# xswang/xflow

Hardware: NVIDIA H100
Metric: training examples/sec (higher is better)
Workload: dtype f32

## Files before the change

xflow_b200/csrc/kernels.cu:

```cuda
#include <cuda_runtime.h>
#include <stdint.h>
#include <stdlib.h>

#include "kernels.h"
#include "table.cuh"

__global__ void xf_k_fill(uint8_t* base, uint64_t cap, uint32_t stride, int lazy) {
  const uint64_t chunks_per_row = stride / 16;
  const uint64_t total = cap * chunks_per_row;
  for (uint64_t c = (uint64_t)blockIdx.x * blockDim.x + threadIdx.x; c < total;
       c += (uint64_t)gridDim.x * blockDim.x) {
    uint64_t r = c / chunks_per_row;
    uint32_t q = (uint32_t)(c % chunks_per_row);
    uint4 v = make_uint4(0, 0, 0, 0);
    if (q == 0) {
      v.x = 0xFFFFFFFFu; v.y = 0xFFFFFFFFu;
      if (!lazy) v.w = XF_NEG_ZERO_BITS;
    }
    *reinterpret_cast<uint4*>(base + r * stride + (uint64_t)q * 16) = v;
  }
}

template <int VEC>
__device__ __forceinline__ void xf_ldv(const float* p, float (&o)[VEC]) {
  if (VEC == 4) { float4 t = __ldcg(reinterpret_cast<const float4*>(p)); o[0] = t.x; o[1 % VEC] = t.y; o[2 % VEC] = t.z; o[3 % VEC] = t.w; }
  else if (VEC == 2) { float2 t = __ldcg(reinterpret_cast<const float2*>(p)); o[0] = t.x; o[1 % VEC] = t.y; }
  else { o[0] = __ldcg(p); }
}
template <int VEC>
__device__ __forceinline__ void xf_stv(float* p, const float (&o)[VEC]) {
  if (VEC == 4) *reinterpret_cast<float4*>(p) = make_float4(o[0], o[1 % VEC], o[2 % VEC], o[3 % VEC]);
  else if (VEC == 2) *reinterpret_cast<float2*>(p) = make_float2(o[0], o[1 % VEC]);
  else *p = o[0];
}
template <int VEC, bool SLOTG, bool STAMP>
__global__ void __launch_bounds__(256)
xf_k_update(XfTableView t, const uint32_t* __restrict__ slots, uint64_t n, int tps, double rows,
            const float* __restrict__ gw, const float* __restrict__ gv, int part,
            unsigned long long* __restrict__ live_total, const uint32_t* __restrict__ n_dev,
            const uint32_t* __restrict__ rows_dev, uint32_t extra_base, uint32_t extra_n,
            const float* __restrict__ v0_side, XfStampView sv) {
  __shared__ unsigned int s_live;
  if (threadIdx.x == 0) s_live = 0;
  __syncthreads();
  uint64_t n_head = n;
  if (n_dev != nullptr) {
    n_head = min((uint64_t)__ldg(n_dev), (uint64_t)extra_base);
    n = n_head + extra_n;
    rows = (double)__ldg(rows_dev);
  }
  unsigned int live_acc = 0;
  const int K = t.K;
  const unsigned lane = threadIdx.x & 31u;
  const uint64_t gwarp = ((uint64_t)blockIdx.x * blockDim.x + threadIdx.x) >> 5;
  const uint64_t nwarps = ((uint64_t)gridDim.x * blockDim.x) >> 5;
  const int q = (int)(lane & (unsigned)(tps - 1));
  const int gi = (int)(lane / (unsigned)tps);
  const int ngroups = 32 / tps;
  const int leader = (int)(lane & ~(unsigned)(tps - 1));
  const unsigned group_mask = (tps == 32) ? 0xffffffffu : (((1u << tps) - 1u) << leader);
  const int nchunk = K / VEC;

  for (uint64_t base = gwarp * 32; base < n; base += nwarps * 32) {
    const uint64_t e_fwd = base + lane;
    const uint64_t e_i = (SLOTG && e_fwd < n) ? (n - 1 - e_fwd) : e_fwd;
    const uint64_t e_phys = (e_i < n_head) ? e_i : (uint64_t)extra_base + (e_i - n_head);
    const uint32_t s_lane = (e_fwd < n) ? __ldcs(slots + e_phys) : 0xFFFFFFFFu;
    unsigned pend = __ballot_sync(0xffffffffu, s_lane != 0xFFFFFFFFu);
    if (live_total != nullptr && lane == 0) live_acc += __popc(pend);

    while (pend) {
      const int cnt = __popc(pend);
      const unsigned src = (gi < cnt) ? __fns(pend, 0, gi + 1) : 0u;
      const uint32_t s = __shfl_sync(0xffffffffu, s_lane, (int)src);
      const uint64_t i = __shfl_sync(0xffffffffu, (unsigned long long)e_i, (int)src);
      const uint64_t i_phys = __shfl_sync(0xffffffffu, (unsigned long long)e_phys, (int)src);
      uint8_t* rowp = (gi < cnt) ? xf_row(t, s) : nullptr;
      pend = (cnt <= ngroups) ? 0u : (pend & ~((2u << __fns(pend, 0, ngroups)) - 1u));

      const bool lat = K > 0 && (part & 2) && rowp != nullptr;
      float* vp = lat ? xf_row_v(rowp) : nullptr;
      float* nvp = lat ? xf_row_nv(rowp, K) : nullptr;
      float* zvp = lat ? xf_row_zv(rowp, K) : nullptr;
      float v0[VEC], n0[VEC], z0[VEC];
#pragma unroll
      for (int e = 0; e < VEC; ++e) { v0[e] = 0.f; n0[e] = 0.f; z0[e] = 0.f; }
      const bool has0 = lat && q < nchunk;
      if (has0) {
        xf_ldv<VEC>(vp + q * VEC, v0);
        if (t.opt == XF_OPT_FTRL) { xf_ldv<VEC>(nvp + q * VEC, n0); xf_ldv<VEC>(zvp + q * VEC, z0); }
      }
      float p0[VEC];
#pragma unroll
      for (int e = 0; e < VEC; ++e) p0[e] = 0.f;
      if (SLOTG && v0_side != nullptr && has0) {
        const uint64_t tok = (i_phys < (uint64_t)extra_base) ? i_phys : (uint64_t)__ldg(slots + i_phys + extra_n);
        xf_ldv<VEC>(v0_side + tok * (uint64_t)K + q * VEC, p0);
      }
      float ca0[VEC];
#pragma unroll
      for (int e = 0; e < VEC; ++e) ca0[e] = 0.f;
      if (SLOTG && t.canon && has0) xf_ldv<VEC>(xf_row_ca(t, rowp) + q * VEC, ca0);
      double accL = 0.0, accA = 0.0;
      if (SLOTG && has0) {
        const double2 a = __ldcg(reinterpret_cast<const double2*>(xf_row_acc(rowp, K)));
        accL = a.x;
        accA = a.y;
      }
      XfHead h;
      h.key = 0; h.flags = 0; h.w = h.n = h.z = 0.f; h.g = 0.0;
      if (q == 0 && rowp != nullptr) h = xf_load_head(rowp);
      const uint64_t key = __shfl_sync(group_mask, (unsigned long long)h.key, leader);
      const uint32_t flags = __shfl_sync(group_mask, h.flags, leader);
      if (rowp == nullptr) continue;

      if (q == 0) {
        if (!SLOTG) xf_apply_pending(t, h);
        if (part & 1) {
          const float g = SLOTG ? xf_div_rows((float)h.g, rows) : gw[i];
          xf_opt_coord(t, g, h.w, h.n, h.z);
        }
        if (SLOTG) h.g = -0.0;
        if (K > 0 && (part & 2)) h.flags |= XF_FLAG_V_READY;
        xf_store_head_t(t, rowp, h);
        if (STAMP) sv.stamp[s] = sv.now;
      }
      if (lat) {
        const bool ready = (flags & XF_FLAG_V_READY) != 0;
        for (int c = q; c < nchunk; c += tps) {
          const int k = c * VEC;
          float v[VEC], g[VEC], nn[VEC], zz[VEC];
#pragma unroll
          for (int e = 0; e < VEC; ++e) { v[e] = v0[e]; nn[e] = n0[e]; zz[e] = z0[e]; }
          if (c != q && ready) {
            xf_ldv<VEC>(vp + k, v);
            if (t.opt == XF_OPT_FTRL) { xf_ldv<VEC>(nvp + k, nn); xf_ldv<VEC>(zvp + k, zz); }
          }
          if (!ready) {
#pragma unroll
            for (int e = 0; e < VEC; ++e) { v[e] = xf_v_init(t, key, (uint32_t)(k + e)); nn[e] = 0.f; zz[e] = 0.f; }
          }
          if (SLOTG) {
            float vp0[VEC];
#pragma unroll
            for (int e = 0; e < VEC; ++e) vp0[e] = v[e];
            if (v0_side != nullptr) {
              if (c == q) {
#pragma unroll
                for (int e = 0; e < VEC; ++e) vp0[e] = p0[e];
              } else {
                const uint64_t tok = (i_phys < (uint64_t)extra_base) ? i_phys : (uint64_t)__ldg(slots + i_phys + extra_n);
                xf_ldv<VEC>(v0_side + tok * (uint64_t)K + k, vp0);
              }
            }
            if (t.canon) {
              float ca[VEC];
#pragma unroll
              for (int e = 0; e < VEC; ++e) ca[e] = ca0[e];
              if (c != q) xf_ldv<VEC>(xf_row_ca(t, rowp) + k, ca);
#pragma unroll
              for (int e = 0; e < VEC; ++e) g[e] = xf_div_rows((float)((double)ca[e] - (double)vp0[e] * accL), rows);
              const float zero[VEC] = {};
              xf_stv<VEC>(xf_row_ca(t, rowp) + k, zero);
            } else {
#pragma unroll
              for (int e = 0; e < VEC; ++e) g[e] = xf_div_rows((float)(accA - (double)vp0[e] * accL), rows);
            }
          } else {
#pragma unroll
            for (int e = 0; e < VEC; ++e) g[e] = gv[i * (uint64_t)K + k + e];
          }
          if (t.opt == XF_OPT_FTRL) {
#pragma unroll
            for (int e = 0; e < VEC; ++e) xf_ftrl_coord(t, g[e], v[e], nn[e], zz[e]);
            xf_stv<VEC>(nvp + k, nn);
            xf_stv<VEC>(zvp + k, zz);
          } else {
#pragma unroll
            for (int e = 0; e < VEC; ++e) xf_sgd_coord(t, g[e], v[e]);
          }
          xf_stv<VEC>(vp + k, v);
        }
        if (SLOTG) {
          __syncwarp(group_mask);
          if (q == 0) *reinterpret_cast<double2*>(xf_row_acc(rowp, K)) = make_double2(0.0, 0.0);
        }
      }
    }
  }
  if (live_total != nullptr) {
    if (lane == 0 && live_acc) atomicAdd(&s_live, live_acc);
    __syncthreads();
    if (threadIdx.x == 0 && s_live) atomicAdd_system(live_total, (unsigned long long)s_live);
  }
}

template <bool INSERT>
__global__ void xf_k_probe(XfTableView t, const uint64_t* __restrict__ keys, uint64_t n,
                           uint32_t* __restrict__ slots, float* __restrict__ w_out, XfStampView sv) {
  for (uint64_t i = (uint64_t)blockIdx.x * blockDim.x + threadIdx.x; i < n;
       i += (uint64_t)gridDim.x * blockDim.x) {
    XfHead h;
    h.w = 0.f;
    int64_t s = xf_probe<INSERT, true>(t, keys[i], &h, &sv);
    slots[i] = s >= 0 ? (uint32_t)s : 0xFFFFFFFFu;
    if (w_out) {
      if (s >= 0) xf_apply_pending(t, h);
      w_out[i] = s >= 0 ? h.w : 0.f;
    }
  }
}

__global__ void xf_k_gather_v(XfTableView t, const uint32_t* __restrict__ slots, const uint64_t* __restrict__ keys,
                              uint64_t n, float* __restrict__ v_out) {
  const int K = t.K;
  const uint64_t total = n * (uint64_t)K;
  for (uint64_t x = (uint64_t)blockIdx.x * blockDim.x + threadIdx.x; x < total;
       x += (uint64_t)gridDim.x * blockDim.x) {
    const uint64_t i = x / K;
    const int k = (int)(x % K);
    const uint32_t s = slots[i];
    float v = 0.f;
    if (s != 0xFFFFFFFFu) {
      const uint8_t* rowp = xf_row(t, s);
      const uint32_t flags = __ldcg(reinterpret_cast<const uint32_t*>(rowp + XF_OFF_FLAGS));
      v = (flags & XF_FLAG_V_READY) ? __ldcg(reinterpret_cast<const float*>(rowp + 32) + k)
                                    : xf_v_init(t, keys[i], (uint32_t)k);
    }
    v_out[x] = v;
  }
}

__global__ void xf_k_import(XfTableView t, const uint32_t* __restrict__ slots, uint64_t n,
                            const float* w, const float* nw, const float* zw, const float* v,
                            const float* nv, const float* zv) {
  const int K = t.K;
  const uint64_t per = (uint64_t)K + 1;
  const uint64_t total = n * per;
  for (uint64_t x = (uint64_t)blockIdx.x * blockDim.x + threadIdx.x; x < total;
       x += (uint64_t)gridDim.x * blockDim.x) {
    const uint64_t i = x / per;
    const int c = (int)(x % per);
    const uint32_t s = slots[i];
    if (s == 0xFFFFFFFFu) continue;
    uint8_t* rowp = xf_row(t, s);
    if (c == 0) {
      if (w) {
        if (t.lazy) {
          XfHead h;
          h.key = *reinterpret_cast<const uint64_t*>(rowp);
          h.w = w[i]; h.n = nw ? nw[i] : 0.f; h.z = zw ? zw[i] : 0.f; h.flags = 0u; h.g = 0.0;
          xf_lazy_store(t, rowp, h, true);
        } else {
          *reinterpret_cast<float2*>(rowp + XF_OFF_STATE) = make_float2(w[i], nw ? nw[i] : 0.f);
          *reinterpret_cast<float*>(rowp + XF_OFF_STATE + 8) = zw ? zw[i] : 0.f;
          *reinterpret_cast<unsigned long long*>(rowp + 8) = XF_NEG_ZERO_BITS64;
        }
      }
      if (v && K > 0) *reinterpret_cast<uint32_t*>(rowp + XF_OFF_FLAGS) = XF_FLAG_V_READY;
    } else if (v) {
      const int k = c - 1;
      xf_row_v(rowp)[k] = v[i * K + k];
      if (k == 0) *reinterpret_cast<double2*>(xf_row_acc(rowp, K)) = make_double2(0.0, 0.0);
      if (t.opt == XF_OPT_FTRL) {
        xf_row_nv(rowp, K)[k] = nv ? nv[i * K + k] : 0.f;
        xf_row_zv(rowp, K)[k] = zv ? zv[i * K + k] : 0.f;
      }
    }
  }
}

__global__ void xf_k_export(XfTableView t, const uint32_t* __restrict__ slots, const uint64_t* __restrict__ keys,
                            uint64_t n, float* w, float* nw, float* zw, float* v, float* nv, float* zv,
                            uint8_t* present) {
  const int K = t.K;
  const uint64_t per = (uint64_t)K + 1;
  const uint64_t total = n * per;
  for (uint64_t x = (uint64_t)blockIdx.x * blockDim.x + threadIdx.x; x < total;
       x += (uint64_t)gridDim.x * blockDim.x) {
    const uint64_t i = x / per;
    const int c = (int)(x % per);
    const uint32_t s = slots[i];
    const bool have = s != 0xFFFFFFFFu;
    const uint8_t* rowp = have ? xf_row(t, s) : nullptr;
    if (c == 0) {
      XfHead h;
      h.w = h.n = h.z = 0.f;
      if (have) {
        h = xf_load_head(rowp);
        xf_apply_pending(t, h);
      }
      if (present) present[i] = have ? 1 : 0;
      if (w) w[i] = h.w;
      if (nw) nw[i] = h.n;
      if (zw) zw[i] = h.z;
    } else if (v) {
      const int k = c - 1;
      float vv = 0.f, nn = 0.f, zz = 0.f;
      if (have) {
        const uint32_t flags = __ldcg(reinterpret_cast<const uint32_t*>(rowp + XF_OFF_FLAGS));
        if (flags & XF_FLAG_V_READY) {
          vv = __ldcg(reinterpret_cast<const float*>(rowp + 32) + k);
          if (t.opt == XF_OPT_FTRL) {
            nn = __ldcg(xf_row_nv(const_cast<uint8_t*>(rowp), K) + k);
            zz = __ldcg(xf_row_zv(const_cast<uint8_t*>(rowp), K) + k);
          }
        } else {
          vv = xf_v_init(t, keys[i], (uint32_t)k);
        }
      }
      v[i * K + k] = vv;
      if (nv) nv[i * K + k] = nn;
      if (zv) zv[i * K + k] = zz;
    }
  }
}

__global__ void xf_k_rehash(XfTableView src, XfTableView dst, XfKeep keep, const uint32_t* __restrict__ src_stamp,
                            uint32_t* __restrict__ dst_stamp) {
  const uint64_t cap = src.mask + 1;
  const uint32_t chunks = src.stride / 16;
  for (uint64_t r = (uint64_t)blockIdx.x * blockDim.x + threadIdx.x; r < cap;
       r += (uint64_t)gridDim.x * blockDim.x) {
    const uint8_t* srow = xf_row(src, r);
    uint4 a = *reinterpret_cast<const uint4*>(srow);
    uint64_t key = (uint64_t)a.x | ((uint64_t)a.y << 32);
    if (key == XF_EMPTY_KEY) continue;
    const uint32_t stamp = src_stamp != nullptr ? src_stamp[r] : 0u;
    if (src_stamp != nullptr && !xf_keeps(keep, stamp, key)) continue;
    XfHead h;
    int64_t s = xf_probe<true>(dst, key, &h);
    if (s < 0) continue;
    uint8_t* drow = xf_row(dst, (uint64_t)s);
    *reinterpret_cast<uint2*>(drow + 8) = make_uint2(a.z, a.w);
    for (uint32_t c = 1; c < chunks; ++c)
      *reinterpret_cast<uint4*>(drow + 16 * c) = *reinterpret_cast<const uint4*>(srow + 16 * c);
    if (dst_stamp != nullptr) dst_stamp[s] = stamp;
  }
}

__global__ void xf_k_list_keys(XfTableView t, uint64_t* keys_out, unsigned long long* count, uint64_t max_out) {
  const uint64_t cap = t.mask + 1;
  for (uint64_t r = (uint64_t)blockIdx.x * blockDim.x + threadIdx.x; r < cap;
       r += (uint64_t)gridDim.x * blockDim.x) {
    const uint64_t key = *reinterpret_cast<const uint64_t*>(xf_row(t, r));
    if (key == XF_EMPTY_KEY) continue;
    unsigned long long idx = atomicAdd(count, 1ull);
    if (idx < max_out) keys_out[idx] = key;
  }
}

static int g_sm_count = 0;
int xf_sms() {
  if (g_sm_count == 0) {
    int dev = 0;
    cudaGetDevice(&dev);
    cudaDeviceGetAttribute(&g_sm_count, cudaDevAttrMultiProcessorCount, dev);
    if (g_sm_count <= 0) g_sm_count = 132;
  }
  return g_sm_count;
}
int xf_grid_for(uint64_t work_items, int block, int blocks_per_sm) {
  uint64_t want = (work_items + block - 1) / block;
  uint64_t cap = (uint64_t)xf_sms() * blocks_per_sm;
  if (want < 1) want = 1;
  return (int)(want < cap ? want : cap);
}

int xf_vec_for(int K) { return K <= 0 ? 1 : (K % 4 == 0 ? 4 : (K % 2 == 0 ? 2 : 1)); }
int xf_tps_for(int K) {
  if (K <= 0) return 1;
  int chunks = K / xf_vec_for(K);
  int tps = 1;
  while (tps < chunks && tps < 32) tps <<= 1;
  return tps;
}

void xf_launch_fill(const XfTableView& t, cudaStream_t st) {
  uint64_t cap = t.mask + 1;
  uint64_t total = cap * (t.stride / 16);
  xf_k_fill<<<xf_grid_for(total, 256, 16), 256, 0, st>>>(t.base, cap, t.stride, t.lazy);
}

template <bool SLOTG, bool STAMP = false>
static void xf_launch_update_t(const XfTableView& t, const uint32_t* slots, uint64_t n, double rows,
                               const float* gw, const float* gv, int part, unsigned long long* live_total,
                               cudaStream_t st, const uint32_t* n_dev = nullptr, const uint32_t* rows_dev = nullptr,
                               uint32_t extra_base = 0, uint32_t extra_n = 0, const float* v0_side = nullptr,
                               XfStampView sv = XfStampView{nullptr, 0u}) {
  const int tps = xf_tps_for(t.K);
  const int grid = xf_grid_for(n * (uint64_t)tps, 256, 8);
#define XF_UPD_ARGS t, slots, n, tps, rows, gw, gv, part, live_total, n_dev, rows_dev, extra_base, extra_n, v0_side, sv
  switch (xf_vec_for(t.K)) {
    case 4: xf_k_update<4, SLOTG, STAMP><<<grid, 256, 0, st>>>(XF_UPD_ARGS); break;
    case 2: xf_k_update<2, SLOTG, STAMP><<<grid, 256, 0, st>>>(XF_UPD_ARGS); break;
    default: xf_k_update<1, SLOTG, STAMP><<<grid, 256, 0, st>>>(XF_UPD_ARGS); break;
  }
#undef XF_UPD_ARGS
}

void xf_launch_update_touched_dev(const XfTableView& t, const uint32_t* touched, uint64_t work_bound,
                                  const uint32_t* n_dev, const uint32_t* rows_dev, uint32_t extra_base,
                                  uint32_t extra_n, const float* v0_side, unsigned long long* unique_total,
                                  cudaStream_t st) {
  xf_launch_update_t<true>(t, touched, work_bound + extra_n, 1.0, nullptr, nullptr, 3, unique_total, st, n_dev, rows_dev,
                           extra_base, extra_n, v0_side);
}

__global__ void xf_k_flush_pending(XfTableView t) {
  const uint64_t cap = t.mask + 1;
  for (uint64_t r = (uint64_t)blockIdx.x * blockDim.x + threadIdx.x; r < cap; r += (uint64_t)gridDim.x * blockDim.x) {
    uint8_t* rowp = xf_row(t, r);
    XfHead h = xf_load_head(rowp);
    if (h.key == XF_EMPTY_KEY || !xf_lazy_has_pending(h)) continue;
    xf_apply_pending(t, h);
    xf_lazy_store(t, rowp, h);
  }
}
void xf_launch_flush_pending(const XfTableView& t, cudaStream_t st) {
  xf_k_flush_pending<<<xf_grid_for(t.mask + 1, 256, 8), 256, 0, st>>>(t);
}

void xf_launch_update_touched(const XfTableView& t, const uint32_t* touched, uint64_t nnz, double rows,
                              unsigned long long* unique_total, const XfStampView& sv, cudaStream_t st) {
  if (nnz == 0) return;
  if (sv.stamp)
    xf_launch_update_t<true, true>(t, touched, nnz, rows, nullptr, nullptr, 3, unique_total, st, nullptr, nullptr, 0, 0,
                                   nullptr, sv);
  else
    xf_launch_update_t<true>(t, touched, nnz, rows, nullptr, nullptr, 3, unique_total, st);
}

void xf_launch_update_pushed(const XfTableView& t, const uint32_t* slots, uint64_t n, const float* gw,
                             const float* gv, cudaStream_t st) {
  if (n == 0) return;
  int part = (gw ? 1 : 0) | (gv ? 2 : 0);
  xf_launch_update_t<false>(t, slots, n, 1.0, gw, gv, part, nullptr, st);
}

void xf_launch_probe(const XfTableView& t, const uint64_t* keys, uint64_t n, bool insert, uint32_t* slots,
                     float* w_out, cudaStream_t st, const XfStampView& sv) {
  if (n == 0) return;
  const int grid = xf_grid_for(n, 256, 8);
  if (insert) xf_k_probe<true><<<grid, 256, 0, st>>>(t, keys, n, slots, w_out, sv);
  else xf_k_probe<false><<<grid, 256, 0, st>>>(t, keys, n, slots, w_out, sv);
}

void xf_launch_gather_v(const XfTableView& t, const uint32_t* slots, const uint64_t* keys, uint64_t n,
                        float* v_out, cudaStream_t st) {
  if (n == 0 || t.K == 0) return;
  xf_k_gather_v<<<xf_grid_for(n * t.K, 256, 8), 256, 0, st>>>(t, slots, keys, n, v_out);
}

void xf_launch_import(const XfTableView& t, const uint32_t* slots, uint64_t n, const float* w, const float* nw,
                      const float* zw, const float* v, const float* nv, const float* zv, cudaStream_t st) {
  if (n == 0) return;
  xf_k_import<<<xf_grid_for(n * (t.K + 1), 256, 8), 256, 0, st>>>(t, slots, n, w, nw, zw, v, nv, zv);
}

void xf_launch_export(const XfTableView& t, const uint32_t* slots, const uint64_t* keys, uint64_t n, float* w,
                      float* nw, float* zw, float* v, float* nv, float* zv, uint8_t* present, cudaStream_t st) {
  if (n == 0) return;
  xf_k_export<<<xf_grid_for(n * (t.K + 1), 256, 8), 256, 0, st>>>(t, slots, keys, n, w, nw, zw, v, nv, zv, present);
}

void xf_launch_rehash(const XfTableView& src, const XfTableView& dst, const XfKeep& keep, const uint32_t* src_stamp,
                      uint32_t* dst_stamp, cudaStream_t st) {
  xf_k_rehash<<<xf_grid_for(src.mask + 1, 256, 8), 256, 0, st>>>(src, dst, keep, src_stamp, dst_stamp);
}

void xf_launch_list_keys(const XfTableView& t, uint64_t* keys_out, unsigned long long* count, uint64_t max_out,
                         cudaStream_t st) {
  xf_k_list_keys<<<xf_grid_for(t.mask + 1, 256, 8), 256, 0, st>>>(t, keys_out, count, max_out);
}
```

Baseline: 92.68 million.

## Specialize touched-row update kernel and prefetch next row into L2

Splits the update kernel into round/load/apply helpers and adds template specializations for the optimizer, side-buffer and canon paths plus a one-chunk-per-thread mode. The touched-row launch now uses a lean variant with the optimizer fixed at compile time, higher launch-bounds occupancy, and a grid sized from measured occupancy. For FTRL it fetches the next row's slot ahead of time and issues an L2 prefetch for it while the current row is applied, aiming to hide random-access memory latency. This adds code complexity, more template instantiations and possible register pressure from the tighter launch bounds.

Result: no change. 92.50 million, median of 6 (-0.2%).

```diff
diff --git a/xflow_b200/csrc/kernels.cu b/xflow_b200/csrc/kernels.cu
--- a/xflow_b200/csrc/kernels.cu
+++ b/xflow_b200/csrc/kernels.cu
@@ -33,13 +33,197 @@
   else if (VEC == 2) *reinterpret_cast<float2*>(p) = make_float2(o[0], o[1 % VEC]);
   else *p = o[0];
 }
-template <int VEC, bool SLOTG, bool STAMP>
-__global__ void __launch_bounds__(256)
+#define XF_OPT_ANY (-1)
+
+template <int OPT>
+__device__ __forceinline__ bool xf_upd_ftrl(const XfTableView& t) {
+  return OPT == XF_OPT_ANY ? t.opt == XF_OPT_FTRL : OPT == XF_OPT_FTRL;
+}
+
+struct XfUpdWalk {
+  uint64_t base;
+  uint64_t e_i, e_phys;
+  uint32_t s_lane;
+  unsigned pend;
+};
+
+struct XfUpdEntry {
+  uint8_t* rowp;
+  uint32_t s;
+  uint64_t i, i_phys;
+};
+template <int VEC>
+struct XfUpdRow {
+  XfUpdEntry e;
+  XfHead h;
+  double accL, accA;
+  float v[VEC], n[VEC], z[VEC];
+  float p[VEC], ca[VEC];
+};
+
+template <bool SLOTG>
+__device__ __forceinline__ bool xf_upd_round(XfUpdWalk& w, XfUpdEntry& r, const XfTableView& t,
+                                             const uint32_t* __restrict__ slots, uint64_t n, uint64_t n_head,
+                                             uint32_t extra_base, uint64_t step, unsigned lane, int gi, int ngroups,
+                                             bool count, unsigned& live_acc) {
+  while (w.pend == 0u) {
+    if (w.base >= n) return false;
+    const uint64_t e_fwd = w.base + lane;
+    w.e_i = (SLOTG && e_fwd < n) ? (n - 1 - e_fwd) : e_fwd;
+    w.e_phys = (w.e_i < n_head) ? w.e_i : (uint64_t)extra_base + (w.e_i - n_head);
+    w.s_lane = (e_fwd < n) ? __ldcs(slots + w.e_phys) : 0xFFFFFFFFu;
+    w.pend = __ballot_sync(0xffffffffu, w.s_lane != 0xFFFFFFFFu);
+    if (count && lane == 0) live_acc += __popc(w.pend);
+    w.base += step;
+  }
+  const int cnt = __popc(w.pend);
+  const unsigned src = (gi < cnt) ? __fns(w.pend, 0, gi + 1) : 0u;
+  r.s = __shfl_sync(0xffffffffu, w.s_lane, (int)src);
+  r.i = __shfl_sync(0xffffffffu, (unsigned long long)w.e_i, (int)src);
+  r.i_phys = __shfl_sync(0xffffffffu, (unsigned long long)w.e_phys, (int)src);
+  r.rowp = (gi < cnt) ? xf_row(t, r.s) : nullptr;
+  w.pend = (cnt <= ngroups) ? 0u : (w.pend & ~((2u << __fns(w.pend, 0, ngroups)) - 1u));
+  return true;
+}
+
+template <int VEC, bool SLOTG, int OPT, bool V0SIDE, bool CANON>
+__device__ __forceinline__ void xf_upd_load(const XfTableView& t, XfUpdRow<VEC>& r, int q, int part,
+                                            const uint32_t* __restrict__ slots, uint32_t extra_base,
+                                            uint32_t extra_n, const float* __restrict__ v0_side) {
+  const int K = t.K;
+  const bool lat = K > 0 && (part & 2) && r.e.rowp != nullptr;
+#pragma unroll
+  for (int e = 0; e < VEC; ++e) { r.v[e] = 0.f; r.n[e] = 0.f; r.z[e] = 0.f; r.p[e] = 0.f; r.ca[e] = 0.f; }
+  const bool has0 = lat && q < K / VEC;
+  if (has0) {
+    xf_ldv<VEC>(xf_row_v(r.e.rowp) + q * VEC, r.v);
+    if (xf_upd_ftrl<OPT>(t)) {
+      xf_ldv<VEC>(xf_row_nv(r.e.rowp, K) + q * VEC, r.n);
+      xf_ldv<VEC>(xf_row_zv(r.e.rowp, K) + q * VEC, r.z);
+    }
+  }
+  if (SLOTG && V0SIDE && v0_side != nullptr && has0) {
+    const uint64_t tok = (r.e.i_phys < (uint64_t)extra_base) ? r.e.i_phys : (uint64_t)__ldg(slots + r.e.i_phys + extra_n);
+    xf_ldv<VEC>(v0_side + tok * (uint64_t)K + q * VEC, r.p);
+  }
+  if (SLOTG && CANON && t.canon && has0) xf_ldv<VEC>(xf_row_ca(t, r.e.rowp) + q * VEC, r.ca);
+  r.accL = 0.0;
+  r.accA = 0.0;
+  if (SLOTG && has0) {
+    const double2 a = __ldcg(reinterpret_cast<const double2*>(xf_row_acc(r.e.rowp, K)));
+    r.accL = a.x;
+    r.accA = a.y;
+  }
+  r.h.key = 0; r.h.flags = 0; r.h.w = r.h.n = r.h.z = 0.f; r.h.g = 0.0;
+  if (q == 0 && r.e.rowp != nullptr) r.h = xf_load_head(r.e.rowp);
+}
+
+template <int VEC, bool SLOTG, bool STAMP, int OPT, bool V0SIDE, bool CANON, bool ONECHUNK>
+__device__ __forceinline__ void xf_upd_apply(const XfTableView& t, XfUpdRow<VEC>& r, int q, int tps, int leader,
+                                             unsigned group_mask, double rows, const float* __restrict__ gw,
+                                             const float* __restrict__ gv, int part, const uint32_t* __restrict__ slots,
+                                             uint32_t extra_base, uint32_t extra_n, const float* __restrict__ v0_side,
+                                             const XfStampView& sv) {
+  const int K = t.K;
+  const bool ftrl = xf_upd_ftrl<OPT>(t);
+  XfHead& h = r.h;
+  const uint64_t key = __shfl_sync(group_mask, (unsigned long long)h.key, leader);
+  const uint32_t flags = __shfl_sync(group_mask, h.flags, leader);
+  uint8_t* rowp = r.e.rowp;
+  if (rowp == nullptr) return;
+
+  if (q == 0) {
+    if (!SLOTG) xf_apply_pending(t, h);
+    if (part & 1) {
+      const float g = SLOTG ? xf_div_rows((float)h.g, rows) : gw[r.e.i];
+      if (ftrl) xf_ftrl_coord(t, g, h.w, h.n, h.z);
+      else xf_sgd_coord(t, g, h.w);
+    }
+    if (SLOTG) h.g = -0.0;
+    if (K > 0 && (part & 2)) h.flags |= XF_FLAG_V_READY;
+    xf_store_head_t(t, rowp, h);
+    if (STAMP) sv.stamp[r.e.s] = sv.now;
+  }
+  if (K > 0 && (part & 2)) {
+    float* vp = xf_row_v(rowp);
+    float* nvp = xf_row_nv(rowp, K);
+    float* zvp = xf_row_zv(rowp, K);
+    const bool ready = (flags & XF_FLAG_V_READY) != 0;
+    auto chunk = [&](int c) {
+      const int k = c * VEC;
+      float v[VEC], g[VEC], nn[VEC], zz[VEC];
+#pragma unroll
+      for (int e = 0; e < VEC; ++e) { v[e] = r.v[e]; nn[e] = r.n[e]; zz[e] = r.z[e]; }
+      if (!ONECHUNK && c != q && ready) {
+        xf_ldv<VEC>(vp + k, v);
+        if (ftrl) { xf_ldv<VEC>(nvp + k, nn); xf_ldv<VEC>(zvp + k, zz); }
+      }
+      if (!ready) {
+#pragma unroll
+        for (int e = 0; e < VEC; ++e) { v[e] = xf_v_init(t, key, (uint32_t)(k + e)); nn[e] = 0.f; zz[e] = 0.f; }
+      }
+      if (SLOTG) {
+        float vp0[VEC];
+#pragma unroll
+        for (int e = 0; e < VEC; ++e) vp0[e] = v[e];
+        if (V0SIDE && v0_side != nullptr) {
+          if (c == q) {
+#pragma unroll
+            for (int e = 0; e < VEC; ++e) vp0[e] = r.p[e];
+          } else {
+            const uint64_t tok = (r.e.i_phys < (uint64_t)extra_base) ? r.e.i_phys : (uint64_t)__ldg(slots + r.e.i_phys + extra_n);
+            xf_ldv<VEC>(v0_side + tok * (uint64_t)K + k, vp0);
+          }
+        }
+        if (CANON && t.canon) {
+          float ca[VEC];
+#pragma unroll
+          for (int e = 0; e < VEC; ++e) ca[e] = r.ca[e];
+          if (c != q) xf_ldv<VEC>(xf_row_ca(t, rowp) + k, ca);
+#pragma unroll
+          for (int e = 0; e < VEC; ++e) g[e] = xf_div_rows((float)((double)ca[e] - (double)vp0[e] * r.accL), rows);
+          const float zero[VEC] = {};
+          xf_stv<VEC>(xf_row_ca(t, rowp) + k, zero);
+        } else {
+#pragma unroll
+          for (int e = 0; e < VEC; ++e) g[e] = xf_div_rows((float)(r.accA - (double)vp0[e] * r.accL), rows);
+        }
+      } else {
+#pragma unroll
+        for (int e = 0; e < VEC; ++e) g[e] = gv[r.e.i * (uint64_t)K + k + e];
+      }
+      if (ftrl) {
+#pragma unroll
+        for (int e = 0; e < VEC; ++e) xf_ftrl_coord(t, g[e], v[e], nn[e], zz[e]);
+        xf_stv<VEC>(nvp + k, nn);
+        xf_stv<VEC>(zvp + k, zz);
+      } else {
+#pragma unroll
+        for (int e = 0; e < VEC; ++e) xf_sgd_coord(t, g[e], v[e]);
+      }
+      xf_stv<VEC>(vp + k, v);
+    };
+    const int nchunk = K / VEC;
+    if (ONECHUNK) {
+      if (q < nchunk) chunk(q);
+    } else {
+      for (int c = q; c < nchunk; c += tps) chunk(c);
+    }
+    if (SLOTG) {
+      __syncwarp(group_mask);
+      if (q == 0) *reinterpret_cast<double2*>(xf_row_acc(rowp, K)) = make_double2(0.0, 0.0);
+    }
+  }
+}
+
+template <int VEC, bool SLOTG, bool STAMP, int OPT, bool V0SIDE, bool CANON, bool ONECHUNK>
+__global__ void __launch_bounds__(256, ((SLOTG && OPT != XF_OPT_ANY && !V0SIDE && !CANON && ONECHUNK) || !SLOTG) ? 3 : 1)
 xf_k_update(XfTableView t, const uint32_t* __restrict__ slots, uint64_t n, int tps, double rows,
             const float* __restrict__ gw, const float* __restrict__ gv, int part,
             unsigned long long* __restrict__ live_total, const uint32_t* __restrict__ n_dev,
             const uint32_t* __restrict__ rows_dev, uint32_t extra_base, uint32_t extra_n,
             const float* __restrict__ v0_side, XfStampView sv) {
+  constexpr bool PIPE = SLOTG && OPT == XF_OPT_FTRL && !V0SIDE && !CANON && ONECHUNK;
   __shared__ unsigned int s_live;
   if (threadIdx.x == 0) s_live = 0;
   __syncthreads();
@@ -50,7 +234,7 @@
     rows = (double)__ldg(rows_dev);
   }
   unsigned int live_acc = 0;
-  const int K = t.K;
+  const bool count = live_total != nullptr;
   const unsigned lane = threadIdx.x & 31u;
   const uint64_t gwarp = ((uint64_t)blockIdx.x * blockDim.x + threadIdx.x) >> 5;
   const uint64_t nwarps = ((uint64_t)gridDim.x * blockDim.x) >> 5;
@@ -59,136 +243,39 @@
   const int ngroups = 32 / tps;
   const int leader = (int)(lane & ~(unsigned)(tps - 1));
   const unsigned group_mask = (tps == 32) ? 0xffffffffu : (((1u << tps) - 1u) << leader);
-  const int nchunk = K / VEC;
-
-  for (uint64_t base = gwarp * 32; base < n; base += nwarps * 32) {
-    const uint64_t e_fwd = base + lane;
-    const uint64_t e_i = (SLOTG && e_fwd < n) ? (n - 1 - e_fwd) : e_fwd;
-    const uint64_t e_phys = (e_i < n_head) ? e_i : (uint64_t)extra_base + (e_i - n_head);
-    const uint32_t s_lane = (e_fwd < n) ? __ldcs(slots + e_phys) : 0xFFFFFFFFu;
-    unsigned pend = __ballot_sync(0xffffffffu, s_lane != 0xFFFFFFFFu);
-    if (live_total != nullptr && lane == 0) live_acc += __popc(pend);
-
-    while (pend) {
-      const int cnt = __popc(pend);
-      const unsigned src = (gi < cnt) ? __fns(pend, 0, gi + 1) : 0u;
-      const uint32_t s = __shfl_sync(0xffffffffu, s_lane, (int)src);
-      const uint64_t i = __shfl_sync(0xffffffffu, (unsigned long long)e_i, (int)src);
-      const uint64_t i_phys = __shfl_sync(0xffffffffu, (unsigned long long)e_phys, (int)src);
-      uint8_t* rowp = (gi < cnt) ? xf_row(t, s) : nullptr;
-      pend = (cnt <= ngroups) ? 0u : (pend & ~((2u << __fns(pend, 0, ngroups)) - 1u));
-
-      const bool lat = K > 0 && (part & 2) && rowp != nullptr;
-      float* vp = lat ? xf_row_v(rowp) : nullptr;
-      float* nvp = lat ? xf_row_nv(rowp, K) : nullptr;
-      float* zvp = lat ? xf_row_zv(rowp, K) : nullptr;
-      float v0[VEC], n0[VEC], z0[VEC];
-#pragma unroll
-      for (int e = 0; e < VEC; ++e) { v0[e] = 0.f; n0[e] = 0.f; z0[e] = 0.f; }
-      const bool has0 = lat && q < nchunk;
-      if (has0) {
-        xf_ldv<VEC>(vp + q * VEC, v0);
-        if (t.opt == XF_OPT_FTRL) { xf_ldv<VEC>(nvp + q * VEC, n0); xf_ldv<VEC>(zvp + q * VEC, z0); }
-      }
-      float p0[VEC];
-#pragma unroll
-      for (int e = 0; e < VEC; ++e) p0[e] = 0.f;
-      if (SLOTG && v0_side != nullptr && has0) {
-        const uint64_t tok = (i_phys < (uint64_t)extra_base) ? i_phys : (uint64_t)__ldg(slots + i_phys + extra_n);
-        xf_ldv<VEC>(v0_side + tok * (uint64_t)K + q * VEC, p0);
-      }
-      float ca0[VEC];
-#pragma unroll
-      for (int e = 0; e < VEC; ++e) ca0[e] = 0.f;
-      if (SLOTG && t.canon && has0) xf_ldv<VEC>(xf_row_ca(t, rowp) + q * VEC, ca0);
-      double accL = 0.0, accA = 0.0;
-      if (SLOTG && has0) {
-        const double2 a = __ldcg(reinterpret_cast<const double2*>(xf_row_acc(rowp, K)));
-        accL = a.x;
-        accA = a.y;
-      }
-      XfHead h;
-      h.key = 0; h.flags = 0; h.w = h.n = h.z = 0.f; h.g = 0.0;
-      if (q == 0 && rowp != nullptr) h = xf_load_head(rowp);
-      const uint64_t key = __shfl_sync(group_mask, (unsigned long long)h.key, leader);
-      const uint32_t flags = __shfl_sync(group_mask, h.flags, leader);
-      if (rowp == nullptr) continue;
-
-      if (q == 0) {
-        if (!SLOTG) xf_apply_pending(t, h);
-        if (part & 1) {
-          const float g = SLOTG ? xf_div_rows((float)h.g, rows) : gw[i];
-          xf_opt_coord(t, g, h.w, h.n, h.z);
-        }
-        if (SLOTG) h.g = -0.0;
-        if (K > 0 && (part & 2)) h.flags |= XF_FLAG_V_READY;
-        xf_store_head_t(t, rowp, h);
-        if (STAMP) sv.stamp[s] = sv.now;
-      }
-      if (lat) {
-        const bool ready = (flags & XF_FLAG_V_READY) != 0;
-        for (int c = q; c < nchunk; c += tps) {
-          const int k = c * VEC;
-          float v[VEC], g[VEC], nn[VEC], zz[VEC];
-#pragma unroll
-          for (int e = 0; e < VEC; ++e) { v[e] = v0[e]; nn[e] = n0[e]; zz[e] = z0[e]; }
-          if (c != q && ready) {
-            xf_ldv<VEC>(vp + k, v);
-            if (t.opt == XF_OPT_FTRL) { xf_ldv<VEC>(nvp + k, nn); xf_ldv<VEC>(zvp + k, zz); }
-          }
-          if (!ready) {
-#pragma unroll
-            for (int e = 0; e < VEC; ++e) { v[e] = xf_v_init(t, key, (uint32_t)(k + e)); nn[e] = 0.f; zz[e] = 0.f; }
-          }
-          if (SLOTG) {
-            float vp0[VEC];
-#pragma unroll
-            for (int e = 0; e < VEC; ++e) vp0[e] = v[e];
-            if (v0_side != nullptr) {
-              if (c == q) {
-#pragma unroll
-                for (int e = 0; e < VEC; ++e) vp0[e] = p0[e];
-              } else {
-                const uint64_t tok = (i_phys < (uint64_t)extra_base) ? i_phys : (uint64_t)__ldg(slots + i_phys + extra_n);
-                xf_ldv<VEC>(v0_side + tok * (uint64_t)K + k, vp0);
-              }
-            }
-            if (t.canon) {
-              float ca[VEC];
-#pragma unroll
-              for (int e = 0; e < VEC; ++e) ca[e] = ca0[e];
-              if (c != q) xf_ldv<VEC>(xf_row_ca(t, rowp) + k, ca);
-#pragma unroll
-              for (int e = 0; e < VEC; ++e) g[e] = xf_div_rows((float)((double)ca[e] - (double)vp0[e] * accL), rows);
-              const float zero[VEC] = {};
-              xf_stv<VEC>(xf_row_ca(t, rowp) + k, zero);
-            } else {
-#pragma unroll
-              for (int e = 0; e < VEC; ++e) g[e] = xf_div_rows((float)(accA - (double)vp0[e] * accL), rows);
-            }
-          } else {
-#pragma unroll
-            for (int e = 0; e < VEC; ++e) g[e] = gv[i * (uint64_t)K + k + e];
-          }
-          if (t.opt == XF_OPT_FTRL) {
-#pragma unroll
-            for (int e = 0; e < VEC; ++e) xf_ftrl_coord(t, g[e], v[e], nn[e], zz[e]);
-            xf_stv<VEC>(nvp + k, nn);
-            xf_stv<VEC>(zvp + k, zz);
-          } else {
-#pragma unroll
-            for (int e = 0; e < VEC; ++e) xf_sgd_coord(t, g[e], v[e]);
-          }
-          xf_stv<VEC>(vp + k, v);
-        }
-        if (SLOTG) {
-          __syncwarp(group_mask);
-          if (q == 0) *reinterpret_cast<double2*>(xf_row_acc(rowp, K)) = make_double2(0.0, 0.0);
-        }
-      }
-    }
-  }
-  if (live_total != nullptr) {
+
+  XfUpdWalk w;
+  w.base = gwarp * 32;
+  w.e_i = w.e_phys = 0;
+  w.s_lane = 0xFFFFFFFFu;
+  w.pend = 0u;
+#define XF_UPD_ROUND(r) \
+  xf_upd_round<SLOTG>(w, r, t, slots, n, n_head, extra_base, nwarps * 32, lane, gi, ngroups, count, live_acc)
+#define XF_UPD_LOAD(r) xf_upd_load<VEC, SLOTG, OPT, V0SIDE, CANON>(t, r, q, part, slots, extra_base, extra_n, v0_side)
+#define XF_UPD_APPLY(r)                                                                                            \
+  xf_upd_apply<VEC, SLOTG, STAMP, OPT, V0SIDE, CANON, ONECHUNK>(t, r, q, tps, leader, group_mask, rows, gw, gv, part, \
+                                                                slots, extra_base, extra_n, v0_side, sv)
+  const bool whole_lines = (t.stride & 127u) == 0u;
+  XfUpdRow<VEC> cur;
+  bool more = XF_UPD_ROUND(cur.e);
+  while (more) {
+    XF_UPD_LOAD(cur);
+    if (PIPE) {
+      XfUpdEntry nxt;
+      more = XF_UPD_ROUND(nxt);
+      if (more && whole_lines && nxt.rowp != nullptr && (uint32_t)q * 128u < t.stride)
+        asm volatile("prefetch.global.L2 [%0];" ::"l"(nxt.rowp + 128 * q));
+      XF_UPD_APPLY(cur);
+      cur.e = nxt;
+    } else {
+      XF_UPD_APPLY(cur);
+      more = XF_UPD_ROUND(cur.e);
+    }
+  }
+#undef XF_UPD_ROUND
+#undef XF_UPD_LOAD
+#undef XF_UPD_APPLY
+  if (count) {
     if (lane == 0 && live_acc) atomicAdd(&s_live, live_acc);
     __syncthreads();
     if (threadIdx.x == 0 && s_live) atomicAdd_system(live_total, (unsigned long long)s_live);
@@ -382,20 +469,52 @@
   xf_k_fill<<<xf_grid_for(total, 256, 16), 256, 0, st>>>(t.base, cap, t.stride, t.lazy);
 }
 
-template <bool SLOTG, bool STAMP = false>
+template <int VEC, bool STAMP, int OPT>
+static int xf_update_ctas_per_sm() {
+  static const int n = [] {
+    int v = 0;
+    if (cudaOccupancyMaxActiveBlocksPerMultiprocessor(&v, xf_k_update<VEC, true, STAMP, OPT, false, false, true>, 256, 0) !=
+            cudaSuccess ||
+        v < 1) {
+      cudaGetLastError();
+      v = 1;
+    }
+    return v;
+  }();
+  return n;
+}
+
+template <bool SLOTG, bool STAMP = false, bool LEAN = false>
 static void xf_launch_update_t(const XfTableView& t, const uint32_t* slots, uint64_t n, double rows,
                                const float* gw, const float* gv, int part, unsigned long long* live_total,
                                cudaStream_t st, const uint32_t* n_dev = nullptr, const uint32_t* rows_dev = nullptr,
                                uint32_t extra_base = 0, uint32_t extra_n = 0, const float* v0_side = nullptr,
                                XfStampView sv = XfStampView{nullptr, 0u}) {
   const int tps = xf_tps_for(t.K);
+  const int vec = xf_vec_for(t.K);
+#define XF_UPD_ARGS t, slots, n, tps, rows, gw, gv, part, live_total, n_dev, rows_dev, extra_base, extra_n, v0_side, sv
+  if constexpr (LEAN) {
+    if (!t.canon && t.K / vec <= 32) {
+      const bool ftrl = t.opt == XF_OPT_FTRL;
+#define XF_UPD_LEAN(V, O) \
+  xf_k_update<V, true, STAMP, O, false, false, true><<<xf_grid_for(n * (uint64_t)tps, 256, xf_update_ctas_per_sm<V, STAMP, O>()), 256, 0, st>>>(XF_UPD_ARGS)
+      switch (vec) {
+        case 4: if (ftrl) XF_UPD_LEAN(4, XF_OPT_FTRL); else XF_UPD_LEAN(4, XF_OPT_SGD); break;
+        case 2: if (ftrl) XF_UPD_LEAN(2, XF_OPT_FTRL); else XF_UPD_LEAN(2, XF_OPT_SGD); break;
+        default: if (ftrl) XF_UPD_LEAN(1, XF_OPT_FTRL); else XF_UPD_LEAN(1, XF_OPT_SGD); break;
+      }
+#undef XF_UPD_LEAN
+      return;
+    }
+  }
   const int grid = xf_grid_for(n * (uint64_t)tps, 256, 8);
-#define XF_UPD_ARGS t, slots, n, tps, rows, gw, gv, part, live_total, n_dev, rows_dev, extra_base, extra_n, v0_side, sv
-  switch (xf_vec_for(t.K)) {
-    case 4: xf_k_update<4, SLOTG, STAMP><<<grid, 256, 0, st>>>(XF_UPD_ARGS); break;
-    case 2: xf_k_update<2, SLOTG, STAMP><<<grid, 256, 0, st>>>(XF_UPD_ARGS); break;
-    default: xf_k_update<1, SLOTG, STAMP><<<grid, 256, 0, st>>>(XF_UPD_ARGS); break;
-  }
+#define XF_UPD_GENERIC(V) xf_k_update<V, SLOTG, STAMP, XF_OPT_ANY, true, true, false><<<grid, 256, 0, st>>>(XF_UPD_ARGS)
+  switch (vec) {
+    case 4: XF_UPD_GENERIC(4); break;
+    case 2: XF_UPD_GENERIC(2); break;
+    default: XF_UPD_GENERIC(1); break;
+  }
+#undef XF_UPD_GENERIC
 #undef XF_UPD_ARGS
 }
 
@@ -425,10 +544,10 @@
                               unsigned long long* unique_total, const XfStampView& sv, cudaStream_t st) {
   if (nnz == 0) return;
   if (sv.stamp)
-    xf_launch_update_t<true, true>(t, touched, nnz, rows, nullptr, nullptr, 3, unique_total, st, nullptr, nullptr, 0, 0,
-                                   nullptr, sv);
+    xf_launch_update_t<true, true, true>(t, touched, nnz, rows, nullptr, nullptr, 3, unique_total, st, nullptr, nullptr, 0,
+                                         0, nullptr, sv);
   else
-    xf_launch_update_t<true>(t, touched, nnz, rows, nullptr, nullptr, 3, unique_total, st);
+    xf_launch_update_t<true, false, true>(t, touched, nnz, rows, nullptr, nullptr, 3, unique_total, st);
 }
 
 void xf_launch_update_pushed(const XfTableView& t, const uint32_t* slots, uint64_t n, const float* gw,
```
